# leggedrobotics/qed-splatter

Measured on AMD Instinct MI355X. Metric: train iters/sec @ 1080p, 500k Gaussians (fwd + loss + bwd + Adam; camera-steps/s over all GPUs), higher is better.
Workload: dtype f32

## Files before the change

### include/qed_splat.h

```cpp
#ifndef QED_SPLAT_H
#define QED_SPLAT_H

#include <stdint.h>

#ifdef __cplusplus
extern "C" {
#endif

#define QED_OK 0
#define QED_E_INVALID_ARG (-1)
#define QED_E_WORKSPACE (-2)
#define QED_E_LAUNCH (-3)
#define QED_E_UNSUPPORTED (-4)

#define QED_TILE 16
#define QED_SPLAT_FLOATS 12
#define QED_METRICS_WS_DOUBLES (10 * 1024)
#define QED_STEP_METRICS_WS_DOUBLES (16 * 1024)
#define QED_LOSS_SUMS_FLOATS (8 + 4 * 1024)
#define QED_VSPLAT_FLOATS 16
#define QED_SH_JAC_FLOATS 10

#define QED_F_ANTIALIASED 1u
#define QED_F_LOG_SCALES 2u
// ... 3 lines not shown
#define QED_F_SH_GRAD_COMPACT 64u
#define QED_F_TIGHT_TILES 32u
#define QED_F_CAMERA_C2W 128u

#define QED_ABI_VERSION 3
int qed_version(void);
const char* qed_last_error(void);

int qed_host_device_pointer(void* host, void** device);
#define QED_STATUS_WORDS 4

int qed_camera_setup(int32_t C, const float* c2w, const float* intrinsics, float* viewmats, float* Ks,
                     void* stream);

int qed_project_fwd(int32_t N, int32_t C, const float* means, const float* quats, const float* scales,
                    const float* opacities, const float* sh0, int32_t sh0_stride, const float* shN,
                    int32_t shN_stride, int32_t sh_degree, const float* viewmats, const float* Ks,
                    int32_t width, int32_t height, int32_t tile_w, int32_t tile_h, float eps2d,
                    float near_plane, float far_plane, float radius_clip, uint32_t flags,
                    int32_t* radii, float* means2d, float* depths, float* conics, float* opac_out,
                    float* colors_out, float* splats, int32_t* tiles_per_gauss, uint64_t* tile_masks,
                    int32_t* block_sums, float* viewmats_out, float* Ks_out, float* sh_jac, void* stream);

int qed_project_bwd(int32_t N, int32_t C, const float* means, const float* quats, const float* scales,
                    const float* opacities, const float* sh0, int32_t sh0_stride, const float* shN,
                    int32_t shN_stride, int32_t sh_degree, const float* viewmats, const float* Ks,
                    int32_t width, int32_t height, float eps2d, uint32_t flags, const int32_t* radii,
                    const float* vsplat, float* v_means, float* v_quats, float* v_scales,
                    float* v_opacities, float* v_sh0, int32_t v_sh0_stride, float* v_shN,
                    int32_t v_shN_stride, float* v_viewmats, const float* sh_jac, void* stream);

int qed_pack_color_grad(int32_t total, const float* vsplat, const float* sh_jac, float* out, void* stream);

int qed_sh_grad_from_views(int32_t N, int32_t n_views, const float* means, const float* viewmats,
                           int64_t viewmat_stride, const float* v_views, int64_t view_stride,
                           int32_t sh_degree, float scale, float* v_sh0, int32_t v_sh0_stride,
                           float* v_shN, int32_t v_shN_stride, void* stream);

int qed_isect_scan(const int32_t* block_sums, int32_t n_blocks, int32_t* block_offsets,
                   int32_t* n_isect, int64_t capacity, int32_t* status, void* stream);
int qed_isect_emit(int32_t N, int32_t C, const float* means2d, const int32_t* radii, const float* depths,
                   const int32_t* tiles_per_gauss, const int32_t* block_offsets, int32_t tile_w,
                   int32_t tile_h, int32_t tile_bits, const int32_t* n_isect, int64_t capacity,
                   uint64_t* keys, int32_t* vals, void* stream);

int64_t qed_sort_workspace_bytes(int64_t capacity);
int qed_sort_pairs(uint64_t* keys, int32_t* vals, uint64_t* keys_alt, int32_t* vals_alt,
                   const int32_t* n_dev, int64_t capacity, int32_t end_bit, void* workspace,
                   int64_t workspace_bytes, int32_t* status, void* stream);

#define QED_BIN_AUTO 0
#define QED_BIN_TWO_STAGE 1
#define QED_BIN_TILE_SORT 2
int64_t qed_bin_workspace_bytes(int64_t n_slots, int64_t capacity);
int qed_bin_tiles(int32_t N, int32_t C, const float* means2d, const int32_t* radii, const float* depths,
                  const int32_t* tiles_per_gauss, const float* splats, const uint64_t* tile_masks,
                  const int32_t* block_sums, int32_t tile_w, int32_t tile_h, int64_t capacity, int32_t mode,
                  int32_t* flatten_ids,
                  int32_t* offsets, int32_t* n_isect, uint64_t* isect_ids, void* workspace,
                  int64_t workspace_bytes, int32_t* status, int32_t* host_words, void* stream);

int qed_tile_offsets(const uint64_t* sorted_keys, const int32_t* n_dev, int64_t capacity, int32_t C,
                     int32_t n_tiles, int32_t tile_bits, int32_t* offsets, void* stream);

typedef struct {
    const float* background;
    float* rgb;
    float* depth;
    float* tile_dmax;
} qed_post_t;
typedef struct {
    const float* background;
    const float* render;
    const float* v_rgb;
    const float* v_depth;
} qed_post_grad_t;
#define QED_CL_TILE_WAVES 1
#define QED_CL_QUADRANT_WAVES 2
#define QED_CL_HALF_AND_HALF 3
#define QED_CL_NO_CULL 4
#define QED_CL_ORDER_READY 8
int qed_composite_fwd(int32_t C, int32_t N, const float* splats, const int32_t* flatten_ids,
                      const int32_t* offsets, int32_t width, int32_t height, int32_t tile_w,
                      int32_t tile_h, int32_t channels, const float* backgrounds, float* render,
                      float* alpha, float* t_final, int32_t* last_ids, int32_t* tile_cost,
                      const int32_t* tile_order, const qed_post_t* post, int32_t launch_flags, void* stream);

int qed_composite_bwd(int32_t C, int32_t N, const float* splats, const int32_t* flatten_ids,
                      const int32_t* offsets, int32_t width, int32_t height, int32_t tile_w,
                      int32_t tile_h, int32_t channels, const float* backgrounds,
                      const float* render_alpha, const float* t_final, const int32_t* last_ids,
                      const float* v_render, const float* v_alpha, float* vsplat, const int32_t* tile_cost, int32_t* order_ws,
                      const qed_post_grad_t* post, int32_t launch_flags, void* stream);

int qed_loss_reduce(int32_t n_pix, int32_t channels, const float* render, const float* alpha,
                    const float* background, const float* gt_rgb, const float* gt_depth,
                    const float* mask, float* sums, void* stream);
int qed_loss_grad(int32_t n_pix, int32_t channels, const float* render, const float* alpha,
                  const float* background, const float* gt_rgb, const float* gt_depth,
                  const float* mask, const float* sums, float rgb_weight, float depth_lambda,
                  float* v_render, float* v_alpha, float* losses, const float* v_rgb_extra,
                  const float* extra_sum, int32_t extra_n, float extra_scale, float extra_offset, void* stream);

int64_t qed_ssim_maps_floats(int32_t height, int32_t width);
int64_t qed_ssim_sum_floats(int32_t height, int32_t width);
int qed_ssim_fwd(int32_t height, int32_t width, int32_t channels, const float* pred, const float* alpha,
// ... 115 lines not shown
```

### qed_splatter_amd/_lib.py

```python
from __future__ import annotations

import ctypes as C
import os
import types
from pathlib import Path

_LIB = None
LIB_PATH = Path(__file__).resolve().parent / "lib" / "libqed_splat.so"

_P = C.c_void_p
_I = C.c_int32
_L = C.c_int64
_F = C.c_float
_U = C.c_uint32
_D = C.c_double
SIGNATURES = {
    "qed_version": (C.c_int, []),
    "qed_last_error": (C.c_char_p, []),
    "qed_camera_setup": (C.c_int, [_I, _P, _P, _P, _P, _P]),
    "qed_project_fwd": (C.c_int, [_I, _I, _P, _P, _P, _P, _P, _I, _P, _I, _I, _P, _P, _I, _I, _I, _I, _F, _F, _F,
                                  _F, _U, _P, _P, _P, _P, _P, _P, _P, _P, _P, _P, _P, _P, _P, _P]),
    "qed_project_bwd": (C.c_int, [_I, _I, _P, _P, _P, _P, _P, _I, _P, _I, _I, _P, _P, _I, _I, _F, _U, _P, _P, _P,
                                  _P, _P, _P, _P, _I, _P, _I, _P, _P, _P]),
    "qed_isect_scan": (C.c_int, [_P, _I, _P, _P, _L, _P, _P]),
# ... 24 lines not shown
    "qed_ssim_maps_floats": (C.c_int64, [_I, _I]),
    "qed_ssim_sum_floats": (C.c_int64, [_I, _I]),
    "qed_ssim_fwd": (C.c_int, [_I, _I, _I, _P, _P, _P, _P, _P, _P, _P, _P]),
    "qed_ssim_fwd_step": (C.c_int, [_I, _I, _I, _P, _P, _P, _P, _P, _P, _P, _P, _L, _P, _P, _P, _P]),
    "qed_ssim_bwd": (C.c_int, [_I, _I, _I, _P, _P, _P, _P, _P, _P, _F, _P, _P, _P]),
    "qed_post_process_fwd": (C.c_int, [_I, _I, _P, _P, _P, _P, _P, _P, _P]),
    "qed_post_process_bwd": (C.c_int, [_I, _I, _P, _P, _P, _P, _P, _P, _P, _P]),
    "qed_image_losses_fwd": (C.c_int, [_I, _P, _P, _P, _P, _P, _F, _F, _P, _I, _F, _F, _P, _P, _P]),
    "qed_image_losses_bwd": (C.c_int, [_I, _P, _P, _P, _P, _P, _P, _F, _F, _P, _P, _I, _P, _P, _P]),
    "qed_loss_grad_ssim": (C.c_int, [_I, _I, _I, _P, _P, _P, _P, _P, _P, _P, _P, _F, _F, _F, _P, _P, _P, _P, _I, _F, _P, _L,
                                     _P, _P]),
    "qed_image_losses_ssim_bwd": (C.c_int, [_I, _I, _P, _P, _P, _P, _P, _P, _P, _F, _F, _F, _P, _P, _P, _P, _P, _L, _P]),
    "qed_adam_step": (C.c_int, [_P, _P, _P, _P, _I, _P, _P, _D, _D, _F, _I, _P, _P]),
    "qed_adam_step_dev": (C.c_int, [_P, _P, _P, _P, _I, _P, _P, _D, _D, _F, _P, _P, _P]),
    "qed_adam_step_sh": (C.c_int, [_P, _P, _P, _P, _I, _P, _P, _P, _D, _D, _F, _I, _P, _I, _F, _F, _I, _I, _I, _P, _I,
                                   _P, _L, _P, _L, _F, _I, _P, _P]),
    "qed_bilagrid_slice_fwd": (C.c_int, [_I, _I, _P, _P, _I, _I, _I, _P, _P]),
    "qed_bilagrid_slice_bwd": (C.c_int, [_I, _I, _P, _P, _I, _I, _I, _P, _P, _P, _P, _P]),
    "qed_bilagrid_tv_fwd": (C.c_int, [_I, _P, _I, _I, _I, _P, _P, _P]),
    "qed_bilagrid_tv_bwd": (C.c_int, [_I, _P, _I, _I, _I, _P, _P, _P]),
}

class Post(C.Structure):
    _fields_ = [("background", C.c_void_p), ("rgb", C.c_void_p), ("depth", C.c_void_p), ("tile_dmax", C.c_void_p)]


class PostGrad(C.Structure):
    _fields_ = [("background", C.c_void_p), ("render", C.c_void_p), ("v_rgb", C.c_void_p), ("v_depth", C.c_void_p)]


class AdamTick(C.Structure):
    _fields_ = [("dev_state", C.c_void_p), ("beta1", C.c_float), ("beta2", C.c_float), ("dev_lr_slot", C.c_void_p),
                ("lr_init", C.c_float), ("lr_final", C.c_float), ("max_steps", C.c_int32), ("skip_flag", C.c_void_p)]


LOSS_SUMS_FLOATS = 8 + 4 * 1024
METRICS_WS_DOUBLES = 10 * 1024
STEP_METRICS_WS_DOUBLES = 16 * 1024
BILAGRID_TV_WS_DOUBLES = 1024
F_ANTIALIASED = 1
F_LOG_SCALES = 2
F_LOGIT_OPAC = 4
F_DEPTH_CHANNEL = 8
F_SIGMOID_COLORS = 16
F_TIGHT_TILES = 32
F_CAMERA_C2W = 128
F_SH_GRAD_COMPACT = 64
SPLAT_FLOATS = 12
VSPLAT_FLOATS = 16
SH_JAC_FLOATS = 10
STATUS_WORDS = 4
TILE = 16
CL_TILE_WAVES, CL_QUADRANT_WAVES, CL_HALF_AND_HALF, CL_NO_CULL, CL_ORDER_READY = 1, 2, 3, 4, 8
BIN_AUTO, BIN_TWO_STAGE, BIN_TILE_SORT = 0, 1, 2


def bin_mode() -> int:
    return {"two": BIN_TWO_STAGE, "til": BIN_TILE_SORT}.get(os.environ.get("QED_BIN_MODE", "")[:3], BIN_AUTO)


def composite_launch_flags() -> int:
    f = {"t": CL_TILE_WAVES, "q": CL_QUADRANT_WAVES, "h": CL_HALF_AND_HALF}.get(
        os.environ.get("QED_COMPOSITE_WAVES", "")[:1], 0)
    if os.environ.get("QED_COMPOSITE_NOCULL", "")[:1] == "1":
        f |= CL_NO_CULL
    return f


class QedSplatError(RuntimeError):
    pass


ABI_VERSION = 3


def load():
    global _LIB
    if _LIB is not None:
        return _LIB
    import torch
    path = Path(os.environ.get("QED_SPLAT_LIB", LIB_PATH))
    if not path.exists():
        raise QedSplatError(
            f"{path} not found: build it with `python -m qed_splatter_amd.build` (hipcc, gfx950). "
            "There is no CPU fallback on the product path.")
    cdll = C.CDLL(str(path))
    ns = {"_cdll": cdll}
    for name, (res, args) in SIGNATURES.items():
        fn = getattr(cdll, name)
        fn.restype = res
        fn.argtypes = args
        ns[name] = _wrap(name, fn) if res is C.c_int and args else fn
    got = int(cdll.qed_version())
    if got != ABI_VERSION:
        raise QedSplatError(f"{path} implements C ABI version {got}, this package binds version {ABI_VERSION} "
                            "(include/qed_splat.h: QED_ABI_VERSION): rebuild it with `python -m qed_splatter_amd.build --force`")
    _LIB = types.SimpleNamespace(**ns)
    return _LIB


def _wrap(name, fn):
    def call(*a):
        if TIMER.active:
            tok = TIMER.begin(name)
            rc = fn(*a)
            TIMER.end(tok)
            return rc
        if MARKERS:
            push, pop = MARKERS
            push(name)
            try:
# ... 74 lines not shown
```

### qed_splatter_amd/csrc/isect.hip

```cpp
#include "qed_common.h"

namespace qed {

constexpr int kScanPer = 32;
__global__ void __launch_bounds__(1024)
isect_scan_kernel(const int* __restrict__ block_sums, int n_blocks, int* __restrict__ block_offsets,
                  int* __restrict__ n_isect, long long capacity, int* __restrict__ status) {
    __shared__ long long wave_tot[16];
    __shared__ long long carry_s;
    const int tid = threadIdx.x, lane = tid & 63, wid = tid >> 6;
    if (tid == 0) carry_s = 0;
    __syncthreads();
    for (int base = 0; base < n_blocks; base += 1024 * kScanPer) {
        const int i0 = base + tid * kScanPer;
        int v[kScanPer];
        const bool vec = (((uintptr_t)block_sums | (uintptr_t)block_offsets) & 15) == 0;
        if (vec && i0 + kScanPer <= n_blocks) {
#pragma unroll
            for (int j = 0; j < kScanPer / 4; ++j) {
                const int4 q = reinterpret_cast<const int4*>(block_sums + i0)[j];
                v[4 * j] = q.x; v[4 * j + 1] = q.y; v[4 * j + 2] = q.z; v[4 * j + 3] = q.w;
            }
        } else {
#pragma unroll
// ... 562 lines not shown
            {
                int c[4], t2 = 0;
#pragma unroll
                for (int w = 0; w < 4; ++w) c[w] = s_cnt[w][tid];
                const int cur = s_base[tid];
#pragma unroll
                for (int w = 0; w < 4; ++w) { s_cnt[w][tid] = cur + t2; t2 += c[w]; }
                __syncthreads();
                s_base[tid] = cur + t2;
            }
            __syncthreads();
            if (valid) {
                const int pos = s_cnt[wid][d] + r;
                vdst[start + pos] = vv;
                if (pass < 3) kdst[start + pos] = kk;
            }
            __syncthreads();
        }
        __threadfence_block();
        __syncthreads();
        ksrc = kdst;
        vsrc = vdst;
    }
}

__global__ void __launch_bounds__(256)
tile_depth_sort_kernel(const int* __restrict__ offsets, const int* __restrict__ vals_in, const float* __restrict__ depths,
                       int* __restrict__ vals_out, unsigned* __restrict__ gk0, unsigned* __restrict__ gk1,
                       int* __restrict__ gv0, int* __restrict__ gv1, int n_tiles_total) {
    __shared__ __attribute__((aligned(16))) uint2 s_kv[4][kTileWaveItems];
    __shared__ __attribute__((aligned(16))) int s_cnt[4][kTileBuckets];
    __shared__ int s_wsum[4], s_skip[4];
    const int lane = threadIdx.x & 63, wid = threadIdx.x >> 6;
    const int tile = blockIdx.x * 4 + wid;
    int start = 0, n = 0;
    if (tile < n_tiles_total) { start = offsets[tile]; n = offsets[tile + 1] - start; }
    if (n >= 1 && n <= kTileWaveItems) tile_sort_wave(start, n, lane, s_kv[wid], s_cnt[wid], vals_in, depths, vals_out);
    if (!__syncthreads_or(n > kTileWaveItems)) return;
    static_assert(sizeof(s_kv) >= kTileSortItems * 8 && sizeof(s_cnt) >= (4 * 256 + 256) * 4, "LDS aliasing");
    unsigned* keys = reinterpret_cast<unsigned*>(&s_kv[0][0]);
    int* vals = reinterpret_cast<int*>(keys + kTileSortItems);
    int (*cnt)[256] = reinterpret_cast<int (*)[256]>(&s_cnt[0][0]);
    int* base = &s_cnt[0][0] + 4 * 256;
    for (int j = 0; j < 4; ++j) {
        const int t = blockIdx.x * 4 + j;
        if (t >= n_tiles_total) break;
        const int s0 = offsets[t], m = offsets[t + 1] - s0;
        if (m <= kTileWaveItems) continue;
        __syncthreads();
        tile_sort_long_run(s0, m, vals_in, depths, vals_out, gk0, gk1, gv0, gv1, keys, vals, cnt, base, s_wsum, s_skip);
    }
}

__global__ void __launch_bounds__(256)
isect_ids_kernel(const unsigned* __restrict__ tile_keys, const int* __restrict__ flatten_ids,
                 const float* __restrict__ depths, const int* __restrict__ n_dev, unsigned long long* __restrict__ out) {
    const int i = blockIdx.x * 256 + threadIdx.x;
    if (i < n_dev[0])
        out[i] = ((unsigned long long)tile_keys[i] << 32) | (unsigned long long)__float_as_uint(depths[flatten_ids[i]]);
}

}

using namespace qed;

static long long align256(long long x) { return (x + 255) & ~255ll; }

static unsigned tile_offsets_grid(long long work) {
    long long g = (work / 4 + 255) / 256;
    if (g > 2048) g = 2048;
    return (unsigned)(g < 1 ? 1 : g);
}

struct BinLayout {
    long long n_slots_dev, keysA0, keysA1, valsA0, valsA1, block_sums, block_offsets, keysB0, keysB1, valsB, sort_ws,
        tk1, tv0, tv1, total;
    long long sort_ws_bytes;
};

static BinLayout bin_layout(long long S, long long cap) {
    BinLayout L;
    long long o = 0;
    const long long nblk = (S + 255) / 256 + 1;
    L.n_slots_dev = o; o += 256;
    L.keysA0 = o; o += align256(4 * S);
    L.keysA1 = o; o += align256(4 * S);
    L.valsA0 = o; o += align256(4 * S);
    L.valsA1 = o; o += align256(4 * S);
    L.block_sums = o; o += align256(4 * nblk);
    L.block_offsets = o; o += align256(4 * nblk);
    L.keysB0 = o; o += align256(4 * cap);
    L.keysB1 = o; o += align256(4 * cap);
    L.valsB = o; o += align256(4 * cap);
    L.sort_ws_bytes = sort32_workspace_bytes(S > cap ? S : cap);
    L.sort_ws = o; o += align256(L.sort_ws_bytes);
    L.tk1 = o; o += align256(4 * cap);
    L.tv0 = o; o += align256(4 * cap);
    L.tv1 = o; o += align256(4 * cap);
    L.total = o;
    return L;
}

extern "C" int64_t qed_bin_workspace_bytes(int64_t n_slots, int64_t capacity) {
    if (n_slots < 0 || capacity < 0) return QED_E_INVALID_ARG;
    return bin_layout(n_slots, capacity).total;
}

extern "C" int qed_bin_tiles(int32_t N, int32_t C, const float* means2d, const int32_t* radii, const float* depths,
                             const int32_t* tiles_per_gauss, const float* splats, const uint64_t* tile_masks,
                             const int32_t* block_sums_in, int32_t tile_w, int32_t tile_h, int64_t capacity,
                             int32_t mode, int32_t* flatten_ids,
                             int32_t* offsets, int32_t* n_isect, uint64_t* isect_ids, void* workspace,
                             int64_t workspace_bytes, int32_t* status, int32_t* host_words, void* stream) {
    QED_REQUIRE(N >= 0 && C >= 1 && tile_w > 0 && tile_h > 0, "bad extents");
    QED_REQUIRE(splats == nullptr || (tile_w <= 1023 && tile_h <= 2047), "packed tile rectangles need tile_w <= 1023");
    QED_REQUIRE(tile_masks == nullptr || splats != nullptr, "tile_masks index the rectangles of the splat records");
    QED_REQUIRE(((uintptr_t)tile_masks & 15) == 0, "tile_masks must be 16-byte aligned");
    QED_REQUIRE(capacity >= 0 && capacity < (1ll << 30), "capacity out of range");
    QED_REQUIRE(offsets && n_isect && status && workspace, "null buffers");
    QED_REQUIRE(((uintptr_t)host_words & 15) == 0, "host_words must be 16-byte aligned");
    const long long S = (long long)C * N;
    QED_REQUIRE(S < (1ll << 30), "too many (camera, Gaussian) slots");
    const long long n_tot = (long long)C * tile_w * tile_h;
    int tile_bits = 1;
    while ((1ll << tile_bits) <= (long long)tile_w * tile_h) ++tile_bits;
    int cam_bits = 0;
    while ((1 << cam_bits) < C) ++cam_bits;
    QED_REQUIRE(tile_bits + cam_bits <= 32, "camera/tile key does not fit 32 bits");
    const BinLayout L = bin_layout(S, capacity);
    if (workspace_bytes < L.total) {
        set_error("qed_bin_tiles: workspace too small (%lld < %lld)", (long long)workspace_bytes, L.total);
        return QED_E_WORKSPACE;
    }
    hipStream_t st = (hipStream_t)stream;
    char* w = (char*)workspace;
    int* n_slots_dev = (int*)(w + L.n_slots_dev);
    unsigned* kA0 = (unsigned*)(w + L.keysA0); unsigned* kA1 = (unsigned*)(w + L.keysA1);
    int* vA0 = (int*)(w + L.valsA0); int* vA1 = (int*)(w + L.valsA1);
    int* block_sums = (int*)(w + L.block_sums);
    unsigned* kB0 = (unsigned*)(w + L.keysB0); unsigned* kB1 = (unsigned*)(w + L.keysB1);
    int* vB = (int*)(w + L.valsB);
    void* sort_ws = w + L.sort_ws;
    if (S == 0 || capacity == 0) {
        hipError_t e = hipMemsetAsync(offsets, 0, (size_t)(n_tot + 1) * 4, st);
        if (e == hipSuccess) e = hipMemsetAsync(n_isect, 0, 4, st);
        if (e == hipSuccess && host_words) e = hipMemsetAsync(host_words, 0, 16, st);
        if (e != hipSuccess) { set_error("qed_bin_tiles: memset failed"); return QED_E_LAUNCH; }
        return QED_OK;
    }
    QED_REQUIRE(means2d && radii && depths && tiles_per_gauss && flatten_ids, "null buffers");
    QED_REQUIRE(mode >= QED_BIN_AUTO && mode <= QED_BIN_TILE_SORT, "unknown binning mode");
    const unsigned gridS = (unsigned)((S + 255) / 256);
    constexpr unsigned kSelfScanMaxBlocks = 16384;
    int* block_offsets = (int*)(w + L.block_offsets);
    auto launch_emit = [&](const int* bsums, const int* order, int* vals_out, unsigned slot_mask = 0xFFFFFFFFu) {
        if (gridS <= kSelfScanMaxBlocks) {
            hipLaunchKernelGGL((isect_emit_kernel<unsigned, true>), dim3(gridS), dim3(256), 0, st, N, C, means2d, radii,
                               depths, tiles_per_gauss, bsums, tile_w, tile_h, tile_bits, n_isect, order, kB0, vals_out,
                               splats, (long long)capacity, status, (const unsigned long long*)tile_masks, slot_mask);
        } else {
            hipLaunchKernelGGL(isect_scan_kernel, dim3(1), dim3(1024), 0, st, bsums, (int)gridS, block_offsets, n_isect,
                               (long long)capacity, status);
            hipLaunchKernelGGL((isect_emit_kernel<unsigned, false>), dim3(gridS), dim3(256), 0, st, N, C, means2d, radii,
                               depths, tiles_per_gauss, (const int*)block_offsets, tile_w, tile_h, tile_bits, n_isect, order,
                               kB0, vals_out, splats, (long long)capacity, status, (const unsigned long long*)tile_masks,
                               slot_mask);
        }
    };
    if (mode == QED_BIN_AUTO) mode = capacity <= 1024 * n_tot ? QED_BIN_TILE_SORT : QED_BIN_TWO_STAGE;
    if (mode == QED_BIN_TILE_SORT) {
        const int* bsums = block_sums_in;
        if (bsums == nullptr) {
            hipLaunchKernelGGL(count_sorted_kernel, dim3(gridS), dim3(256), 0, st, (int)S, (const int*)nullptr,
                               tiles_per_gauss, block_sums);
            bsums = block_sums;
        }
        const int end_bit = tile_bits + cam_bits;
        const int passes = (end_bit + 7) / 8;
        int* v_first = (passes & 1) ? flatten_ids : vB;
        int* v_alt = (passes & 1) ? vB : flatten_ids;
        launch_emit(bsums, (const int*)nullptr, v_first);
        const int which = sort_pairs_u32(kB0, v_first, kB1, v_alt, n_isect, capacity, end_bit, sort_ws, L.sort_ws_bytes,
                                         status, st);
        if (which < 0) return which;
        const unsigned* tile_keys = which ? kB1 : kB0;
        unsigned* k_spare = which ? kB0 : kB1;
        const long long work = capacity > n_tot + 1 ? capacity : n_tot + 1;
        hipLaunchKernelGGL(tile_offsets_kernel<unsigned>, dim3(tile_offsets_grid(work)), dim3(256), 0, st, tile_keys,
                           (const int*)n_isect, (int)n_tot, tile_w * tile_h, tile_bits, offsets, (const int*)status,
                       host_words);
        hipLaunchKernelGGL(tile_depth_sort_kernel, dim3((unsigned)((n_tot + 3) / 4)), dim3(256), 0, st,
                           (const int*)offsets, (const int*)vB, depths, flatten_ids, k_spare, (unsigned*)(w + L.tk1),
                           (int*)(w + L.tv0), (int*)(w + L.tv1), (int)n_tot);
        if (isect_ids != nullptr)
            hipLaunchKernelGGL(isect_ids_kernel, dim3((unsigned)((capacity + 255) / 256)), dim3(256), 0, st, tile_keys,
                               (const int*)flatten_ids, depths, (const int*)n_isect, (unsigned long long*)isect_ids);
        return check_launch("qed_bin_tiles");
    }
    int slot_bits = 1;
    while ((1ll << slot_bits) < S) ++slot_bits;
    if (slot_bits > 28) slot_bits = 32;
    const unsigned slot_mask = slot_bits >= 32 ? 0xFFFFFFFFu : (1u << slot_bits) - 1u;
    hipLaunchKernelGGL(depth_keys_kernel, dim3(gridS), dim3(256), 0, st, (int)S, radii, depths, kA0, vA0, n_slots_dev,
                       tiles_per_gauss, slot_bits);
    int which = sort_pairs_u32(kA0, vA0, kA1, vA1, n_slots_dev, S, 32, sort_ws, L.sort_ws_bytes, status, st);
    if (which < 0) return which;
    const int* order = which ? vA1 : vA0;
    hipLaunchKernelGGL(count_sorted_kernel, dim3(gridS), dim3(256), 0, st, (int)S, order, tiles_per_gauss, block_sums,
                       slot_bits);
    const int end_bit = tile_bits + cam_bits;
    const int passes = (end_bit + 7) / 8;
    int* v_first = (passes & 1) ? vB : flatten_ids;
    int* v_alt = (passes & 1) ? flatten_ids : vB;
    launch_emit((const int*)block_sums, order, v_first, slot_mask);
    which = sort_pairs_u32(kB0, v_first, kB1, v_alt, n_isect, capacity, end_bit, sort_ws, L.sort_ws_bytes, status, st);
    if (which < 0) return which;
    const unsigned* tile_keys = which ? kB1 : kB0;
    const long long work = capacity > n_tot + 1 ? capacity : n_tot + 1;
    hipLaunchKernelGGL(tile_offsets_kernel<unsigned>, dim3(tile_offsets_grid(work)), dim3(256), 0, st, tile_keys,
                       (const int*)n_isect, (int)n_tot, tile_w * tile_h, tile_bits, offsets, (const int*)status,
                       host_words);
    if (isect_ids != nullptr)
// ... 44 lines not shown
```

### qed_splatter_amd/csrc/qed_common.h

```cpp
#pragma once
#include <hip/hip_runtime.h>
#include <stdint.h>
#include <stdio.h>

#include "../../include/qed_splat.h"

namespace qed {

void set_error(const char* fmt, ...);

long long sort32_workspace_bytes(long long capacity);
int sort_pairs_u32(unsigned* keys, int* vals, unsigned* keys_alt, int* vals_alt, const int* n_dev, long long capacity,
                   int end_bit, void* workspace, long long workspace_bytes, int* status, hipStream_t st);

constexpr float kAlphaMax = 0.999f;
constexpr float kAlphaMin = 1.0f / 255.0f;
constexpr float kTMin = 1e-4f;
constexpr float kJacMargin = 0.3f;

constexpr int kWave = 64;

inline int check_launch(const char* what) {
    hipError_t e = hipGetLastError();
    if (e != hipSuccess) {
        set_error("%s: %s", what, hipGetErrorString(e));
        return QED_E_LAUNCH;
    }
    return QED_OK;
}

#define QED_REQUIRE(cond, msg)                                 \
    do {                                                       \
        if (!(cond)) {                                         \
            qed::set_error("%s: %s", __func__, msg);           \
            return QED_E_INVALID_ARG;                          \
        }                                                      \
    } while (0)

__device__ __forceinline__ float sigmoidf_dev(float x) { return 1.0f / (1.0f + __expf(-x)); }

__device__ __forceinline__ void tile_rect(float mx, float my, float radius, int tile_w, int tile_h, int& x0,
                                          int& y0, int& x1, int& y1) {
    const float ts = (float)QED_TILE;
    const float tr = radius / ts, tx = mx / ts, ty = my / ts;
    x0 = min(max(0, (int)floorf(tx - tr)), tile_w);
    y0 = min(max(0, (int)floorf(ty - tr)), tile_h);
    x1 = min(max(0, (int)ceilf(tx + tr)), tile_w);
    y1 = min(max(0, (int)ceilf(ty + tr)), tile_h);
}

__device__ __forceinline__ void tight_tile_rect(float mx, float my, float radius, float a, float b, float c, float tau,
                                                int tile_w, int tile_h, int& x0, int& y0, int& x1, int& y1) {
    const float t = tau * (1.f + 1e-4f) + 1e-2f;
    if (!(t > 0.f)) { x0 = y0 = x1 = y1 = 0; return; }
    const float det = fmaxf(a * c - b * b, 1e-30f);
    const float rx = fminf(radius, sqrtf(2.f * t * c / det) * (1.f + 1e-5f) + 0.01f);
    const float ry = fminf(radius, sqrtf(2.f * t * a / det) * (1.f + 1e-5f) + 0.01f);
    const float ts = (float)QED_TILE;
    x0 = min(max(0, (int)floorf((mx - rx) / ts)), tile_w);
    y0 = min(max(0, (int)floorf((my - ry) / ts)), tile_h);
    x1 = min(max(0, (int)ceilf((mx + rx) / ts)), tile_w);
    y1 = min(max(0, (int)ceilf((my + ry) / ts)), tile_h);
}

__device__ __forceinline__ float edge_min(float h, float bb, float s, float ho, float lo, float hi) {
    const float t = __builtin_amdgcn_fmed3f(s, lo, hi);
// ... 299 lines not shown
```

### qed_splatter_amd/csrc/radix_sort.hip

```cpp
#include "qed_common.h"

namespace qed {

constexpr int kSortThreads = 256;
constexpr int kSortWaves = kSortThreads / 64;
constexpr int kRadixBits = 8;
constexpr int kRadix = 1 << kRadixBits;

template <typename KeyT, int KPT>
struct SortCfg {
    static constexpr int kItems = kSortThreads * KPT;
};

template <typename KeyT>
__device__ __forceinline__ unsigned digit_of(KeyT k, int shift, unsigned mask) {
    return (unsigned)(k >> shift) & mask;
}

template <typename KeyT, int KPT>
__global__ void __launch_bounds__(kSortThreads)
sort_hist_kernel(const KeyT* __restrict__ keys, const int* __restrict__ n_dev, int shift, unsigned mask,
                 int nblocks_max, int* __restrict__ hist) {
    constexpr int kItems = SortCfg<KeyT, KPT>::kItems;
    const int n = n_dev[0];
// ... 293 lines not shown
        hipLaunchKernelGGL((sort_global_hist_kernel<KeyT, P>), dim3(hist_grid), dim3(kSortThreads), 0, st, kin, n_dev,
                           end_bit, ghist);
        for (int p = 0; p < passes; ++p) {
            const int shift = p * kRadixBits;
            const int bits = min(kRadixBits, end_bit - shift);
            const unsigned mask = (1u << bits) - 1u;
            hipLaunchKernelGGL((sort_scatter_kernel<KeyT, KPT, true>), dim3(nblocks_max), dim3(kSortThreads), 0, st, kin,
                               vin, kout, vout, n_dev, shift, mask, nblocks_max, (const int*)nullptr,
                               (const int*)(ghist + p * kRadix), lookback + (size_t)p * nblocks_max * kRadix,
                               tickets + p, status);
            KeyT* tk = kin; kin = kout; kout = tk;
            int* tv = vin; vin = vout; vout = tv;
        }
        const int rc = check_launch("qed_sort_pairs");
        if (rc != QED_OK) return rc;
        return passes & 1;
    }
    const int even_bits = (end_bit + passes - 1) / passes;
    for (int p = 0, shift = 0; p < passes; ++p) {
        const int bits = min(even_bits, end_bit - shift);
        const unsigned mask = (1u << bits) - 1u;
        hipLaunchKernelGGL((sort_hist_kernel<KeyT, KPT>), dim3(nblocks_max), dim3(kSortThreads), 0, st, kin, n_dev,
                           shift, mask, nblocks_max, hist);
        hipLaunchKernelGGL((sort_scan_kernel<kItems>), dim3(kRadix), dim3(kSortThreads), 0, st, n_dev, nblocks_max,
                           hist, digit_tot);
        hipLaunchKernelGGL((sort_scatter_kernel<KeyT, KPT, false>), dim3(nblocks_max), dim3(kSortThreads), 0, st, kin,
                           vin, kout, vout, n_dev, shift, mask, nblocks_max, (const int*)hist, (const int*)digit_tot,
                           (unsigned*)nullptr, (int*)nullptr, (int*)nullptr);
        KeyT* tk = kin; kin = kout; kout = tk;
        int* tv = vin; vin = vout; vout = tv;
        shift += bits;
    }
    const int rc = check_launch("qed_sort_pairs");
    if (rc != QED_OK) return rc;
    return passes & 1;
}

constexpr int kKpt64 = 8;
constexpr int kKpt32 = 8;
constexpr int kKpt32Long = 16;
constexpr long long kSortLongList = 3000000;

long long sort32_workspace_bytes(long long capacity) { return sort_workspace_need<unsigned, kKpt32>(capacity); }

int sort_pairs_u32(unsigned* keys, int* vals, unsigned* keys_alt, int* vals_alt, const int* n_dev, long long capacity,
                   int end_bit, void* workspace, long long workspace_bytes, int* status, hipStream_t st) {
    if (capacity >= kSortLongList)
        return sort_pairs_impl<unsigned, kKpt32Long>(keys, vals, keys_alt, vals_alt, n_dev, capacity, end_bit, workspace,
                                                     workspace_bytes, status, st);
    return sort_pairs_impl<unsigned, kKpt32>(keys, vals, keys_alt, vals_alt, n_dev, capacity, end_bit, workspace,
                                             workspace_bytes, status, st);
}

}

using namespace qed;

extern "C" int64_t qed_sort_workspace_bytes(int64_t capacity) {
    if (capacity < 0) return QED_E_INVALID_ARG;
    return sort_workspace_need<unsigned long long, kKpt64>(capacity);
}

extern "C" int qed_sort_pairs(uint64_t* keys, int32_t* vals, uint64_t* keys_alt, int32_t* vals_alt,
                              const int32_t* n_dev, int64_t capacity, int32_t end_bit, void* workspace,
                              int64_t workspace_bytes, int32_t* status, void* stream) {
    QED_REQUIRE(capacity >= 0 && capacity < (1ll << 31), "capacity out of range");
    QED_REQUIRE(end_bit >= 1 && end_bit <= 64, "end_bit must be in [1, 64]");
    QED_REQUIRE(capacity < (1ll << 30), "capacity must be below 2^30 (30-bit look-back words)");
    if (capacity == 0) return 0;
    QED_REQUIRE(keys && vals && keys_alt && vals_alt && n_dev && workspace && status, "null buffers");
    return sort_pairs_impl<unsigned long long, kKpt64>((unsigned long long*)keys, vals, (unsigned long long*)keys_alt,
                                                      vals_alt, n_dev, capacity, end_bit, workspace, workspace_bytes,
                                                      status, (hipStream_t)stream);
}
```

### qed_splatter_amd/rasterization.py

```python
from __future__ import annotations

import math
import time
import warnings
import weakref
from typing import Dict, Optional, Tuple

import torch
from torch import Tensor

from . import _lib as L


_stream = L.current_stream


def _f32c(t: Tensor, name: str) -> Tensor:
    if t.dtype != torch.float32:
        raise TypeError(f"{name} must be float32, got {t.dtype}")
    if not t.is_cuda:
        raise L.QedSplatError(f"{name} must live on the GPU: this operator has no CPU path")
    return t.contiguous()


# ... 300 lines not shown
def _packed_vsplat(C, N, v_means2d, v_depths, v_conics, v_opac, v_rgb, dev) -> Tensor:
    R = L.VSPLAT_FLOATS
    base = None
    if v_means2d is not None:
        base = _VSPLAT_REGISTRY.get(v_means2d.untyped_storage().data_ptr())

    def is_view(g, col, width):
        if g is None or g.untyped_storage().data_ptr() != base.untyped_storage().data_ptr():
            return False
        want = (N * R, R, 1) if width > 1 else (N * R, R)
        shape = (C, N, width) if width > 1 else (C, N)
        return g.storage_offset() == col and tuple(g.shape) == shape and tuple(g.stride()) == want

    if base is not None and base.numel() == C * N * R and is_view(v_means2d, 0, 2) and is_view(v_conics, 4, 3) \
            and is_view(v_opac, 7, 1) and is_view(v_rgb, 8, 3) and (v_depths is None or is_view(v_depths, 11, 1)):
        return base
    out = torch.zeros(C * N, R, dtype=torch.float32, device=dev)
    if v_means2d is not None:
        out[:, 0:2] = v_means2d.reshape(C * N, 2)
    if v_conics is not None:
        out[:, 4:7] = v_conics.reshape(C * N, 3)
    if v_opac is not None:
        out[:, 7] = v_opac.reshape(C * N)
    if v_rgb is not None:
        out[:, 8:11] = v_rgb.reshape(C * N, 3)
    if v_depths is not None:
        out[:, 11] = v_depths.reshape(C * N)
    return out


def _bin_and_sort(N, C, means2d, radii, depths, tiles_per_gauss, block_sums, tile_w, tile_h, sync=True, splats=None,
                  size=None, tile_masks=None, capture_slot=None):
    lib = L.load()
    dev = means2d.device
    ws = _workspace(dev)
    n_tiles = tile_w * tile_h
    key = (tuple(size) if size is not None else (tile_w, tile_h), N, C)
    n_isect = ws.n_isect
    offsets = torch.empty(C * n_tiles + 1, dtype=torch.int32, device=dev)
    capturing = torch.cuda.is_current_stream_capturing()
    if capturing:
        if ws.capacity == 0 or key not in ws.m_seen:
            raise L.QedSplatError("run one eager call of this shape (image size, number of Gaussians, cameras) before "
                                  "capturing: it calibrates the intersection capacity")
        sync = False
    else:
        ws.poll_pending()
        if not ws.calibrated(key) or not ws.host_words_ok:
            sync = True
    if ws.capacity == 0:
        ws.capacity = max(1 << 16, 8 * C * N)
    mode = L.bin_mode()
    if mode == L.BIN_AUTO and ws.m_seen.get(key, 0) > 0:
        mode = L.BIN_TILE_SORT if int(1.25 * ws.m_seen[key]) <= 1024 * C * n_tiles else L.BIN_TWO_STAGE
    host = host_ptr = None
    if not sync and not capturing:
        host, host_ptr = ws.host_slot()
    elif capturing and capture_slot is not None:
        host, host_ptr = capture_slot
    for _attempt in range(2):
        cap = ws.capacity
        flatten_ids = torch.empty(cap, dtype=torch.int32, device=dev)
        isect_ids = torch.empty(cap, dtype=torch.int64, device=dev) if sync else None
        scratch = torch.empty(int(lib.qed_bin_workspace_bytes(C * N, cap)), dtype=torch.uint8, device=dev)
        L.check(lib.qed_bin_tiles(N, C, L.ptr(means2d), L.ptr(radii), L.ptr(depths), L.ptr(tiles_per_gauss), L.ptr(splats),
                                  L.ptr(tile_masks), L.ptr(block_sums), tile_w, tile_h, cap, mode, L.ptr(flatten_ids), L.ptr(offsets),
                                  L.ptr(n_isect), L.ptr(isect_ids), L.ptr(scratch), scratch.numel(), L.ptr(ws.status),
                                  host_ptr, _stream()), "qed_bin_tiles")
        if capturing:
            ws.last_n_isect = n_isect
            return None, flatten_ids, offsets, None
        if not sync:
            ws.arm_pending(host, key)
            return None, flatten_ids, offsets, None
        host = ws.words[:3].tolist()
        M, overflow = int(host[0]), int(host[1])
        if host[2]:
            ws.status.zero_()
            raise L.QedSplatError("the radix-sort look-back watchdog fired: the list of this frame is mis-sorted")
        if overflow == 0:
            ws.saw(key, M)
            ws.force_sync = False
            return isect_ids[:M], flatten_ids[:M], offsets, M
        ws.status.zero_()
        ws.saw(key, overflow)
    raise L.QedSplatError("intersection buffer overflow persisted after regrowth")


class _Composite(torch.autograd.Function):
    @staticmethod
    def forward(ctx, means2d, conics, rgb, opac, depths, splats, flatten_ids, offsets, backgrounds, width, height,
                tile_w, tile_h, channels, absgrad, vsplat_holder=None, post_background=None, grad_leaf=None,
                tile_order=None):
        lib = L.load()
        ctx.set_materialize_grads(False)
        ctx.vsplat_holder = vsplat_holder
        ctx.grad_leaf = grad_leaf[0] if grad_leaf else None
        ctx.order_slot = tile_order if isinstance(tile_order, list) else None
        if ctx.order_slot is not None:
            tile_order = ctx.order_slot[0] if ctx.order_slot[1] else None
        C, N = opac.shape
        dev = opac.device
        render = torch.empty(C, height, width, channels, dtype=torch.float32, device=dev)
        alpha = torch.empty(C, height, width, 1, dtype=torch.float32, device=dev)
        last_ids = torch.empty(C, height, width, dtype=torch.int32, device=dev)
        bg = _f32c(backgrounds, "backgrounds") if backgrounds is not None else None
        tile_cost = t_final = None
# ... 192 lines not shown
```

Baseline: 1125.

## Add bucket binning mode: one radix pass plus per-bucket LDS partition

Adds a new binning mode that replaces the tile-key sort with a single radix pass on the high key bits. A per-bucket kernel then counting-sorts the low bits in LDS, writing tile offsets and staging values before the existing per-tile depth sort. The aim is fewer global sort passes and less traffic in tile binning. It becomes the default in auto mode whenever the tile plus camera key fits in 16 bits. In exchange it adds a 1024-thread kernel with a large LDS footprint and ballot-based ranking, and buckets larger than the LDS stage write straight to global memory.

Measured after the change: 1142, median of 6. 1.5% higher.

```diff
diff --git a/include/qed_splat.h b/include/qed_splat.h
--- a/include/qed_splat.h
+++ b/include/qed_splat.h
@@ -79,6 +79,7 @@
 #define QED_BIN_AUTO 0
 #define QED_BIN_TWO_STAGE 1
 #define QED_BIN_TILE_SORT 2
+#define QED_BIN_BUCKET 3
 int64_t qed_bin_workspace_bytes(int64_t n_slots, int64_t capacity);
 int qed_bin_tiles(int32_t N, int32_t C, const float* means2d, const int32_t* radii, const float* depths,
                   const int32_t* tiles_per_gauss, const float* splats, const uint64_t* tile_masks,
diff --git a/qed_splatter_amd/_lib.py b/qed_splatter_amd/_lib.py
--- a/qed_splatter_amd/_lib.py
+++ b/qed_splatter_amd/_lib.py
@@ -100,11 +100,12 @@
 STATUS_WORDS = 4
 TILE = 16
 CL_TILE_WAVES, CL_QUADRANT_WAVES, CL_HALF_AND_HALF, CL_NO_CULL, CL_ORDER_READY = 1, 2, 3, 4, 8
-BIN_AUTO, BIN_TWO_STAGE, BIN_TILE_SORT = 0, 1, 2
+BIN_AUTO, BIN_TWO_STAGE, BIN_TILE_SORT, BIN_BUCKET = 0, 1, 2, 3
 
 
 def bin_mode() -> int:
-    return {"two": BIN_TWO_STAGE, "til": BIN_TILE_SORT}.get(os.environ.get("QED_BIN_MODE", "")[:3], BIN_AUTO)
+    return {"two": BIN_TWO_STAGE, "til": BIN_TILE_SORT, "buc": BIN_BUCKET}.get(os.environ.get("QED_BIN_MODE", "")[:3],
+                                                                            BIN_AUTO)
 
 
 def composite_launch_flags() -> int:
diff --git a/qed_splatter_amd/csrc/isect.hip b/qed_splatter_amd/csrc/isect.hip
--- a/qed_splatter_amd/csrc/isect.hip
+++ b/qed_splatter_amd/csrc/isect.hip
@@ -638,6 +638,140 @@
     }
 }
 
+constexpr int kPartThreads = 1024;
+constexpr int kPartWaves = kPartThreads / 64;
+constexpr int kPartRows = 16;
+constexpr int kPartStage = 32768;
+
+__global__ void __launch_bounds__(kPartThreads)
+bucket_partition_kernel(const unsigned* __restrict__ keys, const int* __restrict__ vals, const int* __restrict__ n_dev,
+                        const int* __restrict__ bucket_tot, int low_bits, int tile_bits, int n_tiles,
+                        int n_tiles_total, int* __restrict__ vals_out, unsigned* __restrict__ keys_out,
+                        int* __restrict__ offsets, const int* __restrict__ status, int* __restrict__ host_words) {
+    __shared__ int s_cnt[kPartWaves][256];
+    __shared__ int s_base[256];
+    __shared__ int s_wsum[4][2];
+    __shared__ int s_stage[kPartStage];
+    const int tid = threadIdx.x, lane = tid & 63, wid = tid >> 6;
+    const int b = blockIdx.x;
+    const int n = n_dev[0];
+    if (b == 0 && tid == 0) {
+        offsets[n_tiles_total] = n;
+        if (host_words != nullptr) {
+            *reinterpret_cast<int4*>(host_words) = make_int4(n, status[0], status[1], 0);
+            __threadfence_system();
+        }
+    }
+    const unsigned dmask = (1u << low_bits) - 1u;
+    int before = 0, size = 0;
+    if (tid < 256) {
+        const int t = bucket_tot[tid];
+        before = tid < b ? t : 0;
+        if (tid == b) size = t;
+    }
+#pragma unroll
+    for (int o = 32; o > 0; o >>= 1) { before += __shfl_xor(before, o, 64); size += __shfl_xor(size, o, 64); }
+    if (wid < 4 && lane == 0) { s_wsum[wid][0] = before; s_wsum[wid][1] = size; }
+    for (int i = tid; i < kPartWaves * 256; i += kPartThreads) (&s_cnt[0][0])[i] = 0;
+    __syncthreads();
+    const int start = s_wsum[0][0] + s_wsum[1][0] + s_wsum[2][0] + s_wsum[3][0];
+    const int m = s_wsum[0][1] + s_wsum[1][1] + s_wsum[2][1] + s_wsum[3][1];
+    const int rpw = ((m + 63) / 64 + kPartWaves - 1) / kPartWaves;
+    const int seg0 = min(wid * rpw * 64, m), seg1 = min(seg0 + rpw * 64, m);
+    const unsigned* kin = keys + start;
+    const int* vin = vals + start;
+    unsigned k0[kPartRows];
+    int v0[kPartRows];
+#pragma unroll
+    for (int j = 0; j < kPartRows; ++j) {
+        const int i = seg0 + 64 * j + lane;
+        const int ic = i < seg1 ? i : max(seg1 - 1, 0);
+        k0[j] = seg1 > seg0 ? kin[ic] : 0u;
+        v0[j] = seg1 > seg0 ? vin[ic] : 0;
+    }
+#pragma unroll
+    for (int j = 0; j < kPartRows; ++j)
+        if (seg0 + 64 * j + lane < seg1) atomicAdd(&s_cnt[wid][k0[j] & dmask], 1);
+    for (int r0 = seg0 + 64 * kPartRows; r0 < seg1; r0 += 64 * kPartRows) {
+        unsigned k[kPartRows];
+#pragma unroll
+        for (int j = 0; j < kPartRows; ++j) {
+            const int i = r0 + 64 * j + lane;
+            k[j] = kin[i < seg1 ? i : seg1 - 1];
+        }
+#pragma unroll
+        for (int j = 0; j < kPartRows; ++j)
+            if (r0 + 64 * j + lane < seg1) atomicAdd(&s_cnt[wid][k[j] & dmask], 1);
+    }
+    __syncthreads();
+    int tot = 0, x = 0;
+    if (tid < 256) {
+#pragma unroll
+        for (int w = 0; w < kPartWaves; ++w) { const int c = s_cnt[w][tid]; s_cnt[w][tid] = tot; tot += c; }
+        x = tot;
+#pragma unroll
+        for (int o = 1; o < 64; o <<= 1) {
+            const int y = __shfl_up(x, o, 64);
+            if (lane >= o) x += y;
+        }
+        if (lane == 63) s_wsum[wid][0] = x;
+    }
+    __syncthreads();
+    if (tid < 256) {
+        int wb = 0;
+        for (int w = 0; w < wid; ++w) wb += s_wsum[w][0];
+        const int base = wb + x - tot;
+        s_base[tid] = base;
+        if (tid <= (int)dmask) {
+            const unsigned key = ((unsigned)b << low_bits) | (unsigned)tid;
+            const unsigned t = key & ((1u << tile_bits) - 1u);
+            const long long lin = (long long)(key >> tile_bits) * n_tiles + t;
+            if ((int)t < n_tiles && lin < n_tiles_total) offsets[lin] = start + base;
+        }
+    }
+    __syncthreads();
+    const bool staged = m <= kPartStage;
+    const unsigned long long lt = (1ull << lane) - 1ull;
+    auto place = [&](int r0, const unsigned (&k)[kPartRows], const int (&v)[kPartRows]) {
+#pragma unroll
+        for (int j = 0; j < kPartRows; ++j) {
+            if (r0 + 64 * j >= seg1) break;
+            const bool valid = r0 + 64 * j + lane < seg1;
+            const unsigned d = k[j] & dmask;
+            unsigned long long peers = __ballot(valid);
+            for (int bit = 0; bit < low_bits; ++bit) {
+                const bool on = (d >> bit) & 1u;
+                const unsigned long long bal = __ballot(on);
+                peers &= on ? bal : ~bal;
+            }
+            if (valid) {
+                const int r = s_cnt[wid][d] + __popcll(peers & lt);
+                if ((peers >> lane) == 1ull) s_cnt[wid][d] = r + 1;
+                const int pos = s_base[d] + r;
+                if (staged) s_stage[pos] = v[j];
+                else vals_out[start + pos] = v[j];
+                if (keys_out != nullptr) keys_out[start + pos] = k[j];
+            }
+        }
+    };
+    place(seg0, k0, v0);
+    for (int r0 = seg0 + 64 * kPartRows; r0 < seg1; r0 += 64 * kPartRows) {
+        unsigned k[kPartRows];
+        int v[kPartRows];
+#pragma unroll
+        for (int j = 0; j < kPartRows; ++j) {
+            const int i = r0 + 64 * j + lane;
+            const int ic = i < seg1 ? i : seg1 - 1;
+            k[j] = kin[ic];
+            v[j] = vin[ic];
+        }
+        place(r0, k, v);
+    }
+    if (!staged) return;
+    __syncthreads();
+    for (int i = tid; i < m; i += kPartThreads) vals_out[start + i] = s_stage[i];
+}
+
 __global__ void __launch_bounds__(256)
 isect_ids_kernel(const unsigned* __restrict__ tile_keys, const int* __restrict__ flatten_ids,
                  const float* __restrict__ depths, const int* __restrict__ n_dev, unsigned long long* __restrict__ out) {
@@ -735,7 +869,7 @@
         return QED_OK;
     }
     QED_REQUIRE(means2d && radii && depths && tiles_per_gauss && flatten_ids, "null buffers");
-    QED_REQUIRE(mode >= QED_BIN_AUTO && mode <= QED_BIN_TILE_SORT, "unknown binning mode");
+    QED_REQUIRE(mode >= QED_BIN_AUTO && mode <= QED_BIN_BUCKET, "unknown binning mode");
     const unsigned gridS = (unsigned)((S + 255) / 256);
     constexpr unsigned kSelfScanMaxBlocks = 16384;
     int* block_offsets = (int*)(w + L.block_offsets);
@@ -753,7 +887,38 @@
                                slot_mask);
         }
     };
-    if (mode == QED_BIN_AUTO) mode = capacity <= 1024 * n_tot ? QED_BIN_TILE_SORT : QED_BIN_TWO_STAGE;
+    if (mode == QED_BIN_AUTO) mode = capacity <= 1024 * n_tot ? QED_BIN_BUCKET : QED_BIN_TWO_STAGE;
+    if (mode == QED_BIN_BUCKET && tile_bits + cam_bits > 16) mode = QED_BIN_TILE_SORT;
+    if (mode == QED_BIN_BUCKET) {
+        const int* bsums = block_sums_in;
+        if (bsums == nullptr) {
+            hipLaunchKernelGGL(count_sorted_kernel, dim3(gridS), dim3(256), 0, st, (int)S, (const int*)nullptr,
+                               tiles_per_gauss, block_sums);
+            bsums = block_sums;
+        }
+        launch_emit(bsums, (const int*)nullptr, flatten_ids);
+        const int end_bit = tile_bits + cam_bits;
+        const int low_bits = end_bit > 8 ? end_bit - 8 : 0;
+        const int* bucket_tot = nullptr;
+        int rc = sort_pass_u32(kB0, flatten_ids, kB1, vB, n_isect, capacity, low_bits, end_bit - low_bits, sort_ws,
+                               L.sort_ws_bytes, &bucket_tot, st);
+        if (rc != QED_OK) return rc;
+        const long long max_key = ((long long)(C - 1) << tile_bits) | (long long)(tile_w * tile_h - 1);
+        const unsigned n_buckets = (unsigned)((max_key >> low_bits) + 1);
+        int* v_tiles = (int*)(w + L.tv0);
+        unsigned* k_tiles = isect_ids != nullptr ? (unsigned*)(w + L.tk1) : nullptr;
+        hipLaunchKernelGGL(bucket_partition_kernel, dim3(n_buckets), dim3(kPartThreads), 0, st, (const unsigned*)kB1,
+                           (const int*)vB, (const int*)n_isect, bucket_tot, low_bits, tile_bits, tile_w * tile_h,
+                           (int)n_tot, v_tiles, k_tiles, offsets, (const int*)status, host_words);
+        hipLaunchKernelGGL(tile_depth_sort_kernel, dim3((unsigned)((n_tot + 3) / 4)), dim3(256), 0, st,
+                           (const int*)offsets, (const int*)v_tiles, depths, flatten_ids, kB0, kB1, vB,
+                           (int*)(w + L.tv1), (int)n_tot);
+        if (isect_ids != nullptr)
+            hipLaunchKernelGGL(isect_ids_kernel, dim3((unsigned)((capacity + 255) / 256)), dim3(256), 0, st,
+                               (const unsigned*)k_tiles, (const int*)flatten_ids, depths, (const int*)n_isect,
+                               (unsigned long long*)isect_ids);
+        return check_launch("qed_bin_tiles");
+    }
     if (mode == QED_BIN_TILE_SORT) {
         const int* bsums = block_sums_in;
         if (bsums == nullptr) {
diff --git a/qed_splatter_amd/csrc/qed_common.h b/qed_splatter_amd/csrc/qed_common.h
--- a/qed_splatter_amd/csrc/qed_common.h
+++ b/qed_splatter_amd/csrc/qed_common.h
@@ -12,6 +12,9 @@
 long long sort32_workspace_bytes(long long capacity);
 int sort_pairs_u32(unsigned* keys, int* vals, unsigned* keys_alt, int* vals_alt, const int* n_dev, long long capacity,
                    int end_bit, void* workspace, long long workspace_bytes, int* status, hipStream_t st);
+int sort_pass_u32(const unsigned* kin, const int* vin, unsigned* kout, int* vout, const int* n_dev, long long capacity,
+                  int shift, int bits, void* workspace, long long workspace_bytes, const int** digit_tot,
+                  hipStream_t st);
 
 constexpr float kAlphaMax = 0.999f;
 constexpr float kAlphaMin = 1.0f / 255.0f;
diff --git a/qed_splatter_amd/csrc/radix_sort.hip b/qed_splatter_amd/csrc/radix_sort.hip
--- a/qed_splatter_amd/csrc/radix_sort.hip
+++ b/qed_splatter_amd/csrc/radix_sort.hip
@@ -369,6 +369,42 @@
                                              workspace_bytes, status, st);
 }
 
+template <int KPT>
+static int sort_pass_impl(const unsigned* kin, const int* vin, unsigned* kout, int* vout, const int* n_dev,
+                          long long capacity, int shift, int bits, void* workspace, long long workspace_bytes,
+                          const int** digit_tot_out, hipStream_t st) {
+    constexpr int kItems = SortCfg<unsigned, KPT>::kItems;
+    const int nblocks_max = (int)((capacity + kItems - 1) / kItems);
+    const long long need = sort_workspace_need<unsigned, KPT>(capacity);
+    if (nblocks_max == 0 || workspace_bytes < need) {
+        set_error("sort_pass_u32: empty capacity or workspace too small (%lld < %lld)", workspace_bytes, need);
+        return QED_E_WORKSPACE;
+    }
+    int* hist = (int*)workspace;
+    int* digit_tot = hist + (long long)kRadix * nblocks_max;
+    const unsigned mask = (1u << bits) - 1u;
+    hipLaunchKernelGGL((sort_hist_kernel<unsigned, KPT>), dim3(nblocks_max), dim3(kSortThreads), 0, st, kin, n_dev,
+                       shift, mask, nblocks_max, hist);
+    hipLaunchKernelGGL((sort_scan_kernel<kItems>), dim3(kRadix), dim3(kSortThreads), 0, st, n_dev, nblocks_max, hist,
+                       digit_tot);
+    hipLaunchKernelGGL((sort_scatter_kernel<unsigned, KPT, false>), dim3(nblocks_max), dim3(kSortThreads), 0, st, kin,
+                       vin, kout, vout, n_dev, shift, mask, nblocks_max, (const int*)hist, (const int*)digit_tot,
+                       (unsigned*)nullptr, (int*)nullptr, (int*)nullptr);
+    *digit_tot_out = digit_tot;
+    return check_launch("sort_pass_u32");
+}
+
+int sort_pass_u32(const unsigned* kin, const int* vin, unsigned* kout, int* vout, const int* n_dev, long long capacity,
+                  int shift, int bits, void* workspace, long long workspace_bytes, const int** digit_tot,
+                  hipStream_t st) {
+    if (bits < 1 || bits > kRadixBits) { set_error("sort_pass_u32: 1..8 digit bits"); return QED_E_INVALID_ARG; }
+    if (capacity >= kSortLongList)
+        return sort_pass_impl<kKpt32Long>(kin, vin, kout, vout, n_dev, capacity, shift, bits, workspace,
+                                          workspace_bytes, digit_tot, st);
+    return sort_pass_impl<kKpt32>(kin, vin, kout, vout, n_dev, capacity, shift, bits, workspace, workspace_bytes,
+                                  digit_tot, st);
+}
+
 }
 
 using namespace qed;
diff --git a/qed_splatter_amd/rasterization.py b/qed_splatter_amd/rasterization.py
--- a/qed_splatter_amd/rasterization.py
+++ b/qed_splatter_amd/rasterization.py
@@ -376,7 +376,7 @@
         ws.capacity = max(1 << 16, 8 * C * N)
     mode = L.bin_mode()
     if mode == L.BIN_AUTO and ws.m_seen.get(key, 0) > 0:
-        mode = L.BIN_TILE_SORT if int(1.25 * ws.m_seen[key]) <= 1024 * C * n_tiles else L.BIN_TWO_STAGE
+        mode = L.BIN_BUCKET if int(1.25 * ws.m_seen[key]) <= 1024 * C * n_tiles else L.BIN_TWO_STAGE
     host = host_ptr = None
     if not sync and not capturing:
         host, host_ptr = ws.host_slot()
```
